# ISAE-PNX/SaDVIO

Hardware: AMD Instinct MI355X
Metric: BA iterations/sec (ms/solve in ms_per_solve), 20-KF/8k-landmark window (higher is better)
Workload: dtype f64; 1 GPU; synthetic 20 KF x 8000 landmarks x 40000 reprojection factors (pixel), GN 10 iters (LM step attempts, early exits disabled); windows_per_gpu=1, parallelism=single window, n_kf=20, n_lmk=8000, n_obs=40000, reduced_dim=114

## Files before the change

### sadvio_amd/csrc/ba_types.h

```cpp
#pragma once
#include <stdint.h>

namespace sadvio {

struct SolveOpts {
    int max_num_iterations;
    int jacobi_scaling;
    int max_num_consecutive_invalid_steps;
    int pad;
    double function_tolerance, gradient_tolerance, parameter_tolerance;
    double initial_radius, max_radius, min_radius;
    double min_lm_diagonal, max_lm_diagonal, min_relative_decrease;
    double huber_a;
    double max_time_ticks;
};

struct WinDev {
    int n_kf, n_cam, n_lmk, n_obs;
    int kf_base, cam_base, lmk_base, obs_base;
    int n_free_kf, dpf, Np, Npose;
    long long S_off;
    int red_off;
    int tile_begin, tile_end;
    int prior_begin, prior_end;
// ... 35 lines not shown
    double T_prior[12];
    double inf[6];
};

struct ImuDev {
    int kf_i, kf_j;
    double dt;
    double dR[9], dv[3], dp[3];
    double J_dR_bg[9], J_dv_ba[9], J_dv_bg[9], J_dp_ba[9], J_dp_bg[9];
    double W[81];
    double sa, sg;
    int win, pad;
};
struct SparseDev {
    int type, kf, lmk0, lmk1;
    int win, kf2;
    double T_prior[12], v_prior[3], ba_prior[3], bg_prior[3], delta[3];
    double W[225];
};
struct LineDev {
    double T[12], model[6];
    int col;
    int win;
};
struct LineObsDev {
    int line, kf, cam, win;
    double meas[6];
};
constexpr int LINE_ROW = 4 * 12 + 4 + 2;
constexpr int SPARSE_NE = 136, SPARSE_E_G = 120, SPARSE_E_COST = 135;
constexpr int SPARSE_H = 15 * 15 + 15 + 2;
constexpr int SPARSE_IX = SPARSE_H + SPARSE_NE;
constexpr int SPARSE_COL = SPARSE_IX + SPARSE_NE;
constexpr int SPARSE_J = SPARSE_COL + 16;
constexpr int IMU_J = 9 * 24 + 9;
constexpr int IMU_NE = 355;
constexpr int IMU_E_G = 300, IMU_E_BH = 324, IMU_E_BG = 342, IMU_E_COST = 354;
constexpr int IMU_H = IMU_J + 6;
constexpr int IMU_IX = IMU_H + IMU_NE;
constexpr int IMU_META = IMU_IX + IMU_NE;
constexpr int IMU_ROW = IMU_META + 5;

struct LmState {
    double radius, decrease_factor, x_cost, x_norm, initial_cost;
    int cur;
    int done, termination, iter;
    int n_success, n_unsuccess, n_invalid, pad;
};

struct FinalRec {
    LmState s;
    double fixed_cost;
};

struct IterAcc {
    double lin_cost;
    double cand_cost;
    double mcc;
    double step_norm2;
    double cand_norm2;
    double fixed_cost;
    unsigned long long gmax_bits;
    int chol_fail;
    int time_up;
};

struct TileAcc {
    double lin_cost, fixed_cost, gmax;
    double cand_cost, mcc, step_norm2, cand_norm2;
    double pad;
};

constexpr int BUILD_THREADS = 256;
constexpr int BUILD_WAVES = BUILD_THREADS / 64;
constexpr int MAX_TILE_KF = 24;
constexpr int MAX_TILE_FREE_KF = 20;
constexpr int MAX_GEMM_FREE_KF = 5;
constexpr int MAX_WIN_CAM = 8;
constexpr int STAGE_VALS = 18;
constexpr int MAX_LMK_OBS = 64;
constexpr int SOLVE_THREADS = 512;
constexpr int SOLVE_KFC_STRIDE = 32;
constexpr int SOLVE_KFC = 32;
constexpr int PRIOR_LIN = 28;
constexpr int PRE_KF = 8;
constexpr int PRE_MAX_TILES = 1024;
constexpr int MAX_LDS_NP = 174;

}
```

### sadvio_amd/csrc/device_math.h

```cpp
#pragma once
#include <hip/hip_runtime.h>

namespace sadvio {

struct V3 {
    double x, y, z;
};

__device__ __forceinline__ void m3_mul(const double* A, const double* B, double* C) {
#pragma unroll
    for (int i = 0; i < 3; i++)
#pragma unroll
        for (int j = 0; j < 3; j++) C[3 * i + j] = A[3 * i] * B[j] + A[3 * i + 1] * B[3 + j] + A[3 * i + 2] * B[6 + j];
}
__device__ __forceinline__ void m3_vec(const double* A, const double* v, double* o) {
    double x = A[0] * v[0] + A[1] * v[1] + A[2] * v[2];
    double y = A[3] * v[0] + A[4] * v[1] + A[5] * v[2];
    double z = A[6] * v[0] + A[7] * v[1] + A[8] * v[2];
    o[0] = x; o[1] = y; o[2] = z;
}
__device__ __forceinline__ void m3_tvec(const double* A, const double* v, double* o) {
    double x = A[0] * v[0] + A[3] * v[1] + A[6] * v[2];
    double y = A[1] * v[0] + A[4] * v[1] + A[7] * v[2];
    double z = A[2] * v[0] + A[5] * v[1] + A[8] * v[2];
// ... 131 lines not shown
__device__ __forceinline__ void li_vec(const double* Li, const double* t, double* u) {
    u[0] = Li[0] * t[0];
    u[1] = Li[1] * t[0] + Li[2] * t[1];
    u[2] = Li[3] * t[0] + Li[4] * t[1] + Li[5] * t[2];
}
__device__ __forceinline__ void li_tvec(const double* Li, const double* u, double* v) {
    v[0] = Li[0] * u[0] + Li[1] * u[1] + Li[3] * u[2];
    v[1] = Li[2] * u[1] + Li[4] * u[2];
    v[2] = Li[5] * u[2];
}
__device__ __forceinline__ void m3_inverse(const double* A, double* I) {
    double c00 = A[4] * A[8] - A[5] * A[7];
    double c01 = A[5] * A[6] - A[3] * A[8];
    double c02 = A[3] * A[7] - A[4] * A[6];
    double id = 1.0 / (A[0] * c00 + A[1] * c01 + A[2] * c02);
    I[0] = c00 * id; I[1] = (A[2] * A[7] - A[1] * A[8]) * id; I[2] = (A[1] * A[5] - A[2] * A[4]) * id;
    I[3] = c01 * id; I[4] = (A[0] * A[8] - A[2] * A[6]) * id; I[5] = (A[2] * A[3] - A[0] * A[5]) * id;
    I[6] = c02 * id; I[7] = (A[1] * A[6] - A[0] * A[7]) * id; I[8] = (A[0] * A[4] - A[1] * A[3]) * id;
}

__device__ __forceinline__ void relative_pose_factor(const double* Ta, const double* Tb, const double* Tab, const double* W,
                                                     const double* da, const double* db, double* r, double* J) {
    double Ea[9], Eb[9], Rau[9], Rbu[9], tau[3], tbu[3], v[3];
    so3_exp(da, Ea); so3_exp(db, Eb);
    m3_mul(Ta, Ea, Rau); m3_mul(Tb, Eb, Rbu);
    m3_vec(Ta, da + 3, v); for (int i = 0; i < 3; i++) tau[i] = v[i] + Ta[9 + i];
    m3_vec(Tb, db + 3, v); for (int i = 0; i < 3; i++) tbu[i] = v[i] + Tb[9 + i];
    double RaT_Rb[9], R[9], d[3], u[3], t[3], w[3];
    m3_tmul(Rau, Rbu, RaT_Rb);
    m3_tmul(Tab, RaT_Rb, R);
    for (int i = 0; i < 3; i++) d[i] = tbu[i] - tau[i];
    m3_tvec(Rau, d, u);
    for (int i = 0; i < 3; i++) u[i] -= Tab[9 + i];
    m3_tvec(Tab, u, t);
    so3_log(R, w);
    const double e[6] = {w[0], w[1], w[2], t[0], t[1], t[2]};
    for (int i = 0; i < 6; i++) { double s = 0.0; for (int j = 0; j < 6; j++) s += W[6 * i + j] * e[j]; r[i] = s; }
    if (!J) return;
    double Jrw[9], Jrwi[9], Jra[9], Jrb[9], A[9], B[9], C[9], S[9], D1[9], D2[9], D3[9], D4[9], E2[9], F[9];
    so3_right_jacobian(w, Jrw); m3_inverse(Jrw, Jrwi);
    so3_right_jacobian(da, Jra); so3_right_jacobian(db, Jrb);
    m3_tmul(Rbu, Rau, A); m3_mul(Jrwi, A, B); m3_mul(B, Jra, C);
    so3_skew(d, S);
    for (int i = 0; i < 3; i++) for (int j = 0; j < 3; j++) { double s = 0.0; for (int k = 0; k < 3; k++) s += Tab[3 * k + i] * Rau[3 * j + k]; D1[3 * i + j] = s; }
    m3_mul(D1, S, D2); m3_mul(D2, Rau, D3); m3_mul(D3, Jra, D4);
    m3_mul(Jrwi, Jrb, E2);
    m3_mul(D1, Rbu, F);
    double Jf[72];
    for (int i = 0; i < 72; i++) Jf[i] = 0.0;
    for (int i = 0; i < 3; i++)
        for (int j = 0; j < 3; j++) {
            Jf[i * 12 + j] = -C[3 * i + j];
            Jf[(3 + i) * 12 + j] = D4[3 * i + j];
            Jf[(3 + i) * 12 + 3 + j] = -Tab[3 * j + i];
            Jf[i * 12 + 6 + j] = E2[3 * i + j];
            Jf[(3 + i) * 12 + 9 + j] = F[3 * i + j];
        }
    for (int i = 0; i < 6; i++)
        for (int c = 0; c < 15; c++) {
            double s = 0.0;
            if (c < 12) for (int k = 0; k < 6; k++) s += W[6 * i + k] * Jf[k * 12 + c];
            J[i * 15 + c] = s;
        }
}

constexpr int POSE_TAB = 42;
__device__ __forceinline__ void pose_table_entry(const double* T0, const double* d6, double* tab) {
    double dR[9], Jr[9], R[9], t[3];
    so3_exp(d6, dR);
    so3_right_jacobian(d6, Jr);
    m3_mul(T0, dR, R);
    m3_vec(T0, d6 + 3, t);
#pragma unroll
    for (int i = 0; i < 9; i++) {
        tab[i] = R[i];
        tab[12 + i] = Jr[i];
        tab[21 + i] = T0[i];
        tab[30 + i] = dR[i];
    }
    tab[9] = t[0] + T0[9]; tab[10] = t[1] + T0[10]; tab[11] = t[2] + T0[11];
    tab[39] = d6[3]; tab[40] = d6[4]; tab[41] = d6[5];
}

template <bool WANT_J>
__device__ __forceinline__ void p2l_pseudo_obs(const double* tab, const double* q, const double* delta, const double* W, int half,
                                               double* r, double* Jp, double* Jl) {
    double Rq[3], e[3];
    m3_vec(tab, q, Rq);
    for (int a = 0; a < 3; a++) e[a] = Rq[a] + tab[9 + a] - delta[a];
    const int r0 = half ? 2 : 0;
    r[0] = W[3 * r0] * e[0] + W[3 * r0 + 1] * e[1] + W[3 * r0 + 2] * e[2];
    r[1] = half ? 0.0 : W[3] * e[0] + W[4] * e[1] + W[5] * e[2];
    if (WANT_J) {
        double Sq[9], A[9], B[9], C[9], WR0[9], WR[9];
        so3_skew(q, Sq);
        m3_mul(tab + 30, Sq, A);
        m3_mul(A, tab + 12, B);
        m3_mul(W, tab + 21, WR0);
        m3_mul(WR0, B, C);
        m3_mul(W, tab, WR);
#pragma unroll
        for (int j = 0; j < 3; j++) {
            Jp[j] = -C[3 * r0 + j]; Jp[3 + j] = WR0[3 * r0 + j]; Jl[j] = WR[3 * r0 + j];
            Jp[6 + j] = half ? 0.0 : -C[3 + j]; Jp[9 + j] = half ? 0.0 : WR0[3 + j]; Jl[3 + j] = half ? 0.0 : WR[3 + j];
        }
    }
}

template <bool WANT_J>
__device__ __forceinline__ bool pixel_factor(const double* tab, const double* K, const double* Tsf, const double* pw,
                                             double u_meas, double v_meas, double inv_sigma, double* r, double* Jp,
                                             double* Jl) {
    double pf[3], tc[3];
    m3_vec(tab, pw, pf);
    pf[0] += tab[9]; pf[1] += tab[10]; pf[2] += tab[11];
    m3_vec(Tsf, pf, tc);
    tc[0] += Tsf[9]; tc[1] += Tsf[10]; tc[2] += Tsf[11];
    double iz = 1.0 / tc[2];
    double u = (K[0] * tc[0] + K[2] * tc[2]) * iz;
    double v = (K[1] * tc[1] + K[3] * tc[2]) * iz;
    bool valid = !(tc[2] < 0.1) && !(u < 0 || v < 0 || u > 2 * K[2] || v > 2 * K[3]) && isfinite(u) && isfinite(v);
    r[0] = valid ? inv_sigma * (u - u_meas) : 0.0;
    r[1] = valid ? inv_sigma * (v - v_meas) : 0.0;
    if (WANT_J) {
        double a0 = inv_sigma * K[0] * iz, a1 = inv_sigma * K[1] * iz;
        double JhK[6] = {a0, 0.0, -a0 * tc[0] * iz, 0.0, a1, -a1 * tc[1] * iz};
        double A[6];
#pragma unroll
        for (int j = 0; j < 3; j++) {
            A[j] = JhK[0] * Tsf[j] + JhK[2] * Tsf[6 + j];
            A[3 + j] = JhK[4] * Tsf[3 + j] + JhK[5] * Tsf[6 + j];
        }
#pragma unroll
        for (int q = 0; q < 2; q++)
#pragma unroll
            for (int j = 0; j < 3; j++) Jl[3 * q + j] = A[3 * q] * tab[j] + A[3 * q + 1] * tab[3 + j] + A[3 * q + 2] * tab[6 + j];
        const double* Jr = tab + 12;
        const double* R0 = tab + 21;
#pragma unroll
        for (int q = 0; q < 2; q++) {
            double l0 = Jl[3 * q], l1 = Jl[3 * q + 1], l2 = Jl[3 * q + 2];
            double s0 = l1 * pw[2] - l2 * pw[1];
            double s1 = l2 * pw[0] - l0 * pw[2];
            double s2 = l0 * pw[1] - l1 * pw[0];
#pragma unroll
            for (int j = 0; j < 3; j++) {
                Jp[6 * q + j] = -(s0 * Jr[j] + s1 * Jr[3 + j] + s2 * Jr[6 + j]);
                Jp[6 * q + 3 + j] = A[3 * q] * R0[j] + A[3 * q + 1] * R0[3 + j] + A[3 * q + 2] * R0[6 + j];
            }
        }
    }
    return valid;
}

template <bool WANT_J>
__device__ __forceinline__ void angular_factor(const double* tab, const double* Tsf, const double* pw,
                                               const double* b, double inv_sigma, double* r, double* Jp, double* Jl) {
    const double* R0 = tab + 21;
    const double* dR = tab + 30;
    double pf[3], ts[3];
    m3_vec(tab, pw, pf);
    pf[0] += tab[9]; pf[1] += tab[10]; pf[2] += tab[11];
    m3_vec(Tsf, pf, ts);
    ts[0] += Tsf[9]; ts[1] += Tsf[10]; ts[2] += Tsf[11];
    double nrm = v3_norm(ts);
    double inrm = 1.0 / nrm;
// ... 388 lines not shown
```

### sadvio_amd/csrc/kernels.h

```cpp
#pragma once
#include "ba_types.h"
#include "device_math.h"
#include "chol16.h"

namespace sadvio {

struct DevPtrs {
    const WinDev* win;
    const Tile* tiles;
    const double* kf_T0;
    const int* kf_fidx;
    double* xp; double* xv; double* xba; double* xbg;
    long long xp_stride, xv_stride, xl_stride;
    const double* kf_vel; const double* kf_ba; const double* kf_bg;
    const double* cam_K; const double* cam_T; const double* cam_isig;
    const double* lmk_p; double* xl; double* s_lmk;
    const unsigned char* lmk_const;
    const int* lmk_ob; const int* lmk_oe;
    const int* obs_kf; const int* obs_cam; const double* obs_meas;
    const unsigned char* obs_slot;
    const int* tile_kf;
    const int* tile_row;
    const int4* pre_lane;
    const int2* pre_kf;
// ... 1119 lines not shown
                                              const double* xba, const double* xbg, const double* xl, const double* y,
                                              double* r, double* J) {
    const int fi = f.kf >= 0 ? P.kf_fidx[f.kf] : -1;
    const int lr0 = sparse_lr0(P, W, f);
    const int lr1 = (f.lmk1 >= 0 && P.lmk_red) ? P.lmk_red[f.lmk1] : -1;
    if (fi < 0 && lr0 < 0 && lr1 < 0) return false;
    const int dpf = W.dpf;
    if (f.type == 5) {
        double da[6], db[6];
        for (int q = 0; q < 6; q++) {
            da[q] = xp[6 * (long long)f.kf + q] + ((y && fi >= 0) ? y[fi * dpf + q] : 0.0);
            db[q] = xp[6 * (long long)f.kf2 + q] + ((y && lr0 >= 0) ? y[lr0 + q] : 0.0);
        }
        relative_pose_factor(P.kf_T0 + 12 * (long long)f.kf, P.kf_T0 + 12 * (long long)f.kf2, f.T_prior, f.W, da, db, r, J);
        return true;
    }
    if (f.type == 0) {
        double prm[15];
        const long long k = f.kf;
        for (int q = 0; q < 6; q++) prm[q] = xp[6 * k + q] + ((y && fi >= 0) ? y[fi * dpf + q] : 0.0);
        for (int q = 0; q < 3; q++) {
            const bool st = y && fi >= 0 && dpf == 15;
            prm[6 + q] = xv[3 * k + q] + (st ? y[fi * 15 + 6 + q] : 0.0);
            prm[9 + q] = xba[3 * k + q] + (st ? y[fi * 15 + 9 + q] : 0.0);
            prm[12 + q] = xbg[3 * k + q] + (st ? y[fi * 15 + 12 + q] : 0.0);
        }
        if (INL) imu_prior_factor_body(P.kf_T0 + 12 * k, P.kf_vel + 3 * k, P.kf_ba + 3 * k, P.kf_bg + 3 * k, f.T_prior, f.v_prior,
                                       f.ba_prior, f.bg_prior, f.W, prm, r, J);
        else imu_prior_factor(P.kf_T0 + 12 * k, P.kf_vel + 3 * k, P.kf_ba + 3 * k, P.kf_bg + 3 * k, f.T_prior, f.v_prior,
                              f.ba_prior, f.bg_prior, f.W, prm, r, J);
        return true;
    }
    double q0[3], q1[3] = {0.0, 0.0, 0.0};
    for (int a = 0; a < 3; a++) {
        q0[a] = P.lmk_p[3 * (long long)f.lmk0 + a] + xl[3 * (long long)f.lmk0 + a] + ((y && lr0 >= 0) ? y[lr0 + a] : 0.0);
        if (f.type == 3) q1[a] = P.lmk_p[3 * (long long)f.lmk1 + a] + xl[3 * (long long)f.lmk1 + a] + ((y && lr1 >= 0) ? y[lr1 + a] : 0.0);
    }
    if (f.type == 1) {
        double d6[6];
        for (int q = 0; q < 6; q++) d6[q] = xp[6 * (long long)f.kf + q] + ((y && fi >= 0) ? y[fi * dpf + q] : 0.0);
        pose_to_landmark_factor(P.kf_T0 + 12 * (long long)f.kf, q0, f.delta, f.W, d6, r, J);
        return true;
    }
    double e[3];
    for (int a = 0; a < 3; a++) e[a] = q0[a] - q1[a] - f.delta[a];
    m3_vec(f.W, e, r);
    if (J) {
        for (int i = 0; i < 3; i++)
            for (int j = 0; j < 3; j++) { J[i * 15 + j] = f.W[3 * i + j]; J[i * 15 + 3 + j] = -f.W[3 * i + j]; }
    }
    return true;
}

__device__ __noinline__ bool sparse_eval(const DevPtrs& P, const WinDev& W, const SparseDev& f, const double* xp, const double* xv,
                                        const double* xba, const double* xbg, const double* xl, const double* y,
                                        double* r, double* J) {
    return sparse_eval_t<false>(P, W, f, xp, xv, xba, xbg, xl, y, r, J);
}


__device__ __forceinline__ double prior_lin_record(const double* T0, const double* Tp, const double* inf, const double* d6, double* rec) {
    double r[6], J[36];
    pose_prior_factor(T0, Tp, inf, d6, r, J);
    double c = 0.0;
#pragma unroll
    for (int a = 0; a < 6; a++) {
        c += r[a] * r[a];
        double g = 0.0;
#pragma unroll
        for (int q = 0; q < 6; q++) g += J[6 * q + a] * r[q];
        rec[a] = g;
#pragma unroll
        for (int b = 0; b <= a; b++) {
            double hh = 0.0;
#pragma unroll
            for (int q = 0; q < 6; q++) hh += J[6 * q + a] * J[6 * q + b];
            rec[6 + a * (a + 1) / 2 + b] = hh;
        }
    }
    rec[27] = c;
    return c;
}

__device__ __noinline__ void pose_table_store(const double* T0, double d0, double d1, double d2, double d3, double d4, double d5, double* dst) {
    double T0r[12], tab[POSE_TAB];
#pragma unroll
    for (int i = 0; i < 12; i++) T0r[i] = T0[i];
    const double d6[6] = {d0, d1, d2, d3, d4, d5};
    pose_table_entry(T0r, d6, tab);
#pragma unroll
    for (int i = 0; i < POSE_TAB; i++) dst[i] = tab[i];
}
__device__ __noinline__ double prior_lin_record_call(const double* T0, double d0, double d1, double d2, double d3, double d4, double d5, const PriorDev* pr,
                                                     double* rec) {
    double T0r[12];
#pragma unroll
    for (int i = 0; i < 12; i++) T0r[i] = T0[i];
    const double d6[6] = {d0, d1, d2, d3, d4, d5};
    const PriorDev q = *pr;
    return prior_lin_record(T0r, q.T_prior, q.inf, d6, rec);
}

template <int MODE, bool EXTRAS>
__global__ __launch_bounds__(SOLVE_THREADS) void k_solve(DevPtrs P, int slot) {
    extern __shared__ __attribute__((aligned(16))) char smem[];
    constexpr bool BIG = MODE != 0;
    const int w = blockIdx.x;
    const WinDev W = P.win[w];
    if (BIG != (W.ld != 0)) return;
    const int tid = threadIdx.x;
    const int wv = __builtin_amdgcn_readfirstlane(tid >> 6), ln = tid & 63, nwv = blockDim.x >> 6;
    LmState* stp = P.states + (long long)w * P.state_stride + slot;
    IterAcc* acc = P.acc + (long long)w * P.state_stride + slot;
    __shared__ int s_done;
    __shared__ double s_red[SOLVE_THREADS / 64 * 4];
    SADVIO_TS(3, 0);
#ifdef SADVIO_KERNEL_TS
    if ((P.debug & 4096) && blockIdx.x == 0 && tid == 0 && slot == 3) P.dbg_ts[20] = clock64();
#endif
    LmState st = *stp;
    if (MODE == 1 && tid == 0) P.big_info[w] = 0;
    if (st.done) return;
    const int Np = W.Np;
    const long long ld = W.ld;
    double* Sg = P.S + W.S_off;
    double* gredg = P.gred + W.red_off;
    double* gfullg = P.gfull + W.red_off;
    double* hdg = P.hdiag + W.red_off;
    const int nbt = c16_blocks(Np + 1);
    const int img_n = c16_size(Np);
    double* A = BIG ? Sg : (double*)smem;
    double* y = BIG ? gredg : A + img_n;
    double* gf = BIG ? gfullg : y + Np;
    double* hd = BIG ? hdg : gf + Np;
    double* xs = BIG ? gredg : hd + Np;
    double* pub = xs + Np + (Np & 1);
    double* yv = pub + C16_WORK;
    double* kfc = yv + 16 * nbt;
    auto aidx = [&](int i, int j) -> long long { return BIG ? (long long)i * ld + j : (long long)c16_index(i, j); };
    const int cur = st.cur;
    const double* xp = P.xp + (long long)cur * P.xp_stride;
    const int n_imu = W.imu_end - W.imu_begin;
    double early_cost = 0.0, early_fixed = 0.0, early_gm = 0.0;
    double cost_part = 0.0, fixed_part = 0.0;
    const int n_pri = W.prior_end - W.prior_begin;
    const double* plin = P.prior_lin + (long long)cur * P.prior_lin_stride + (long long)W.prior_begin * PRIOR_LIN;
    double pl_v = 0.0;
    int pl_fi = -1;
    if (MODE != 2 && tid < n_pri * 28) {
        const int p = tid / 28, e = tid - 28 * p;
        pl_v = plin[p * PRIOR_LIN + e];
        pl_fi = P.kf_fidx[P.priors[W.prior_begin + p].kf];
    }
    double* sp = P.s_pose + W.red_off;
    double c_sp = 1.0;
    const bool det = P.world > 1;
    if (MODE != 2) {
    double im_ix[8], im_v[8];
    const int n_imu_items = (EXTRAS && !det && !P.imu_direct) ? n_imu * IMU_NE : 0;
    if (EXTRAS) {
#pragma unroll
        for (int u = 0; u < 8; u++) {
            const int it = tid + u * (int)blockDim.x;
            im_ix[u] = -1.0; im_v[u] = 0.0;
            if (it < n_imu_items) {
                const int k = it / IMU_NE, e = it - IMU_NE * k;
                const double* row = P.imu_scratch + (long long)cur * P.imu_scratch_stride + (long long)(W.imu_begin + k) * IMU_ROW;
                im_ix[u] = row[IMU_IX + e]; im_v[u] = row[IMU_H + e];
            }
        }
    }
    if (!BIG) {
        typedef __attribute__((address_space(3))) void lds_void_t;
        typedef __attribute__((address_space(1))) const void glb_void_t;
// ... 232 lines not shown
        if (tid < Np) {
            gm = fmax(gm, fabs(gf[tid]));
            const double hdi = hd[tid];
            double s = c_sp;
            if (slot == 0) { s = P.o.jacobi_scaling ? 1.0 / (1.0 + sqrt(hdi)) : 1.0; sp[tid] = s; }
            const double s2 = s * s;
            A[c16_index(tid, tid)] += fmin(fmax(s2 * hdi, P.o.min_lm_diagonal), P.o.max_lm_diagonal) / st.radius / s2;
            A[c16_index(Np, tid)] = y[tid];
        }
    } else {
        for (int i = tid; i < Np; i += blockDim.x) gm = fmax(gm, fabs(gf[i]));
    }
    gm = wave_max(gm); cost_part = wave_sum(cost_part); fixed_part = wave_sum(fixed_part);
    if (ln == 0) { s_red[wv * 3] = gm; s_red[wv * 3 + 1] = cost_part; s_red[wv * 3 + 2] = fixed_part; }
    if (tid == 0) s_done = 0;
    __syncthreads();
    if (!BIG) c16_symmetrize(A, nbt);
    if (tid == blockDim.x - 1) {
        double g = 0, cs = 0, fs = 0;
        for (int k = 0; k < nwv; k++) { g = fmax(g, s_red[k * 3]); cs += s_red[k * 3 + 1]; fs += s_red[k * 3 + 2]; }
        acc->gmax_bits = (unsigned long long)__double_as_longlong(g);
        acc->lin_cost = cs;
        acc->fixed_cost = fs;
        acc->cand_cost = 0.0; acc->mcc = 0.0; acc->step_norm2 = 0.0; acc->cand_norm2 = 0.0;
        const bool time_up = P.o.max_time_ticks > 0.0 && P.t_start && (double)(wall_clock64() - *P.t_start) >= P.o.max_time_ticks;
        acc->time_up = time_up ? 1 : 0;
        const bool no_iterations = st.iter == 0 && P.o.max_num_iterations <= 0;
        if (time_up || g <= P.o.gradient_tolerance || no_iterations) {
            LmState e = st;
            e.done = 1; e.termination = (time_up || g > P.o.gradient_tolerance) ? 0 : 3;
            e.x_cost = 0.5 * cs;
            if (e.iter == 0) e.initial_cost = e.x_cost;
            *stp = e;
            s_done = 1;
        }
    }
    __syncthreads();
    if (s_done) return;
    SADVIO_TS(3, 2);
    if (BIG) {
        for (int i = tid; i < Np; i += blockDim.x) {
            double s;
            if (slot == 0) { s = P.o.jacobi_scaling ? 1.0 / (1.0 + sqrt(hd[i])) : 1.0; sp[i] = s; }
            else s = sp[i];
            double s2 = s * s;
            A[aidx(i, i)] += fmin(fmax(s2 * hd[i], P.o.min_lm_diagonal), P.o.max_lm_diagonal) / st.radius / s2;
        }
        __syncthreads();
    }
    SADVIO_TS(3, 3);
    if (MODE == 1) return;
    }
    long long* ts = SADVIO_TS_PTR((P.debug & 4096) && blockIdx.x == 0 && slot == 3);
    if (MODE == 0) {
        bool ok = true;
        if (Np > 0) ok = c16_solve<1>(A, Np, xs, pub, yv, ts ? ts + 64 : nullptr);
        if (!ok) {
            if (tid == 0) acc->chol_fail = 1;
            return;
        }
    } else {
        y = P.delta + W.red_off;
        if (P.big_info[w] != 0) {
            for (int i = tid; i < Np; i += blockDim.x) { gredg[i] = 0.0; gfullg[i] = 0.0; hdg[i] = 0.0; }
            if (tid == 0) acc->chol_fail = 1;
            return;
        }
    }
    SADVIO_TS(3, 4);
    double* dl = P.delta + W.red_off;
    double sn = 0.0, cn = 0.0;
    bool bad = false;
    for (int i = tid; i < Np; i += blockDim.x) {
        double d = -xs[i];
        dl[i] = d;
        y[i] = d;
        sn += d * d;
        if (!isfinite(d)) bad = true;
        if (BIG) { gredg[i] = 0.0; gfullg[i] = 0.0; hdg[i] = 0.0; }
    }
    __syncthreads();
    SADVIO_TS(3, 5);
    double* xpc = P.xp + (long long)(1 - cur) * P.xp_stride;
    for (int k = tid; k < W.n_kf; k += blockDim.x) {
        int g = W.kf_base + k;
        const bool pre = MODE == 0 && k < SOLVE_KFC;
        const double* kc = kfc + (pre ? k : 0) * SOLVE_KFC_STRIDE;
        int fi = pre ? (int)kc[0] : P.kf_fidx[g];
        double d6[6];
        const double* T0r = pre ? kc + 7 : P.kf_T0 + 12 * (long long)g;
        double vbb[9];
        if (W.dpf == 15) {
            const double* xs3[3] = {P.xv + (long long)cur * P.xv_stride, P.xba + (long long)cur * P.xv_stride, P.xbg + (long long)cur * P.xv_stride};
#pragma unroll
            for (int q = 0; q < 3; q++)
#pragma unroll
                for (int i = 0; i < 3; i++) vbb[3 * q + i] = pre ? kc[19 + 3 * q + i] : xs3[q][3 * (long long)g + i];
        }
#pragma unroll
        for (int i = 0; i < 6; i++) {
            double v = (pre ? kc[1 + i] : xp[6 * (long long)g + i]) + (fi < 0 ? 0.0 : y[fi * W.dpf + i]);
            xpc[6 * (long long)g + i] = v;
            d6[i] = v;
            if (fi >= 0) cn += v * v;
        }
        pose_table_store(T0r, d6[0], d6[1], d6[2], d6[3], d6[4], d6[5], P.ptab + (long long)(1 - cur) * P.ptab_stride + (long long)g * POSE_TAB);
        if (W.dpf == 15) {
            double* xs3[3] = {P.xv + (long long)(1 - cur) * P.xv_stride, P.xba + (long long)(1 - cur) * P.xv_stride, P.xbg + (long long)(1 - cur) * P.xv_stride};
#pragma unroll
            for (int q = 0; q < 3; q++)
#pragma unroll
                for (int i = 0; i < 3; i++) {
                    const double v = vbb[3 * q + i] + (fi < 0 ? 0.0 : y[fi * 15 + 6 + 3 * q + i]);
                    xs3[q][3 * (long long)g + i] = v;
                    if (fi >= 0) cn += v * v;
                }
        }
    }
    if (EXTRAS && W.line_end > W.line_begin) {
        const double* xlc = P.xline + (long long)cur * P.xline_stride;
        double* xln = P.xline + (long long)(1 - cur) * P.xline_stride;
        for (int it = tid; it < (W.line_end - W.line_begin) * 6; it += blockDim.x) {
            const int l = W.line_begin + it / 6, q = it % 6;
            const int lc = P.lines[l].col;
            const double v = xlc[6 * (long long)l + q] + (lc < 0 ? 0.0 : y[lc + q]);
            xln[6 * (long long)l + q] = v;
            if (lc >= 0) cn += v * v;
        }
    }
    SADVIO_TS(3, 6);
    double mcc = 0.0, cc = 0.0;
    {
        const double* plx = P.prior_lin + (long long)cur * P.prior_lin_stride + (long long)W.prior_begin * PRIOR_LIN;
        double* plc = P.prior_lin + (long long)(1 - cur) * P.prior_lin_stride + (long long)W.prior_begin * PRIOR_LIN;
        for (int p = (int)blockDim.x - 1 - tid; p < W.prior_end - W.prior_begin; p += blockDim.x) {
            const PriorDev* prp = P.priors + W.prior_begin + p;
            const int pkf = prp->kf;
            const int fi = P.kf_fidx[pkf];
            if (fi < 0) continue;
            double d[6], d6[6];
#pragma unroll
            for (int i = 0; i < 6; i++) { d[i] = y[fi * W.dpf + i]; d6[i] = xp[6 * (long long)pkf + i] + d[i]; }
            double lin = 0.0, quad = 0.0;
#pragma unroll
            for (int a = 0; a < 6; a++) {
                lin += d[a] * plx[p * PRIOR_LIN + a];
#pragma unroll
                for (int b = 0; b <= a; b++) quad += (a == b ? 0.5 : 1.0) * d[a] * d[b] * plx[p * PRIOR_LIN + 6 + a * (a + 1) / 2 + b];
            }
            mcc += -(lin + quad);
            cc += prior_lin_record_call(P.kf_T0 + 12 * (long long)pkf, d6[0], d6[1], d6[2], d6[3], d6[4], d6[5], prp, plc + p * PRIOR_LIN);
        }
    }
    if (EXTRAS && n_imu > 0) {
        const double* xv = P.xv + (long long)cur * P.xv_stride;
        const double* xba = P.xba + (long long)cur * P.xv_stride;
        const double* xbg = P.xbg + (long long)cur * P.xv_stride;
        const int t0 = blockDim.x > 128 ? 64 : 0;
        for (int it = tid - t0; it >= 0 && it < n_imu * 15; it += blockDim.x - t0) {
            const int k = it / 15, q = it - 15 * k;
            const double* sc = P.imu_scratch + (long long)cur * P.imu_scratch_stride + (long long)(W.imu_begin + k) * IMU_ROW;
            const int fi = (int)sc[IMU_META], fj = (int)sc[IMU_META + 1];
            if (fi < 0 && fj < 0) continue;
            double m = 0.0, r;
            if (q < 9) {
                double jr[24];
#pragma unroll
                for (int a = 0; a < 24; a++) jr[a] = sc[q * 24 + a];
                r = sc[9 * 24 + q];
#pragma unroll
                for (int a = 0; a < 24; a++) { const int ca = imu_col(a, fi, fj); if (ca >= 0) m += jr[a] * y[ca]; }
            } else {
                const int e = q - 9, ax = e % 3, gy = e / 3;
                const double sgm = sc[IMU_META + 2 + gy];
                r = sc[IMU_J + e];
                if (fi >= 0) m -= sgm * y[fi * 15 + 9 + 3 * gy + ax];
                if (fj >= 0) m += sgm * y[fj * 15 + 9 + 3 * gy + ax];
            }
            mcc += -m * (r + 0.5 * m);
        }
    }
    if (EXTRAS && W.spl_end > W.spl_begin) {
        const int t0 = blockDim.x > 320 ? 256 : 0;
        for (int it = tid - t0; it >= 0 && it < (W.spl_end - W.spl_begin) * 15; it += blockDim.x - t0) {
            const int kl = it / 15, q = it - 15 * kl;
            const double* sc = P.sp_scratch + (long long)cur * P.sp_scratch_stride + (long long)P.sp_list[W.spl_begin + kl] * SPARSE_J;
            if (q >= (int)sc[SPARSE_COL + 15]) continue;
            double jr[15], cd[15];
#pragma unroll
            for (int a = 0; a < 15; a++) { jr[a] = sc[q * 15 + a]; cd[a] = sc[SPARSE_COL + a]; }
            const double r = sc[225 + q];
            double m = 0.0;
#pragma unroll
            for (int a = 0; a < 15; a++) { const int ca = (int)cd[a]; if (ca >= 0) m += jr[a] * y[ca]; }
            mcc += -m * (r + 0.5 * m);
        }
    }
    if (EXTRAS && W.lobs_end > W.lobs_begin) {
        const int rows = W.factor_type == 0 ? 4 : 2;
        for (int it = tid; it < (W.lobs_end - W.lobs_begin) * 4; it += blockDim.x) {
            const int k = it >> 2, q = it & 3;
            if (q >= rows) continue;
            const LineObsDev& ob = P.lobs[W.lobs_begin + k];
            const int fi = P.kf_fidx[ob.kf], lc = P.lines[ob.line].col;
            if (fi < 0 && lc < 0) continue;
            const double* sc = P.line_scratch + (long long)(W.lobs_begin + k) * LINE_ROW;
            double m = 0.0;
            for (int a = 0; a < 6; a++) {
                if (fi >= 0) m += sc[q * 12 + a] * y[fi * W.dpf + a];
                if (lc >= 0) m += sc[q * 12 + 6 + a] * y[lc + a];
            }
            mcc += -m * (sc[48 + q] + 0.5 * m);
        }
    }
    SADVIO_TS(3, 7);
    sn = wave_sum(sn); cn = wave_sum(cn); mcc = wave_sum(mcc); cc = wave_sum(cc);
    if (bad) acc->chol_fail = 1;
    __syncthreads();
    if (ln == 0) { s_red[wv * 4] = sn; s_red[wv * 4 + 1] = cn; s_red[wv * 4 + 2] = mcc; s_red[wv * 4 + 3] = cc; }
    __syncthreads();
    if (tid == 0) {
        double a0 = 0, a1 = 0, a2 = 0, a3 = 0;
        for (int k = 0; k < nwv; k++) { a0 += s_red[k * 4]; a1 += s_red[k * 4 + 1]; a2 += s_red[k * 4 + 2]; a3 += s_red[k * 4 + 3]; }
        acc->step_norm2 = a0; acc->cand_norm2 = a1; acc->mcc = a2; acc->cand_cost = a3;
    }
    SADVIO_TS(3, 8);
    if (ts && tid == 0) { ts[15] = wall_clock64(); ts[21] = clock64(); }
}


__device__ __forceinline__ void zero_s_slice(const DevPtrs& P, const Tile& T, int tile_index) {
    if (T.ld != 0) return;
    const int n2 = c16_size(T.Np) >> 1;
    const int per = (n2 + T.win_ntiles - 1) / T.win_ntiles;
    const int i0 = (tile_index - T.win_tile0) * per, i1 = min(i0 + per, n2);
    double2* S2 = (double2*)(P.S + T.S_off);
    const double2 z2 = make_double2(0.0, 0.0);
    for (int i = i0 + (int)threadIdx.x; i < i1; i += blockDim.x) S2[i] = z2;
}

template <int FACTOR, bool RARE, bool IMU>
__global__ __launch_bounds__(BUILD_THREADS) void k_backsub(DevPtrs P, int slot, int max_tile_kf) {
    extern __shared__ __attribute__((aligned(16))) char smem[];
    if (IMU && (int)blockIdx.x >= P.n_tiles) {
        if (threadIdx.x < 64) pose_factor_eval<true>(P, slot, (int)blockIdx.x - P.n_tiles, threadIdx.x);
        return;
    }
    const Tile T = P.tiles[blockIdx.x];
    const int tid = threadIdx.x, wv = tid >> 6, ln = tid & 63;
    int4 pl = make_int4(0, -1, 0, 0);
    int2 pk = make_int2(-1, -1), pk6 = make_int2(-1, -1);
    if (P.pre_lane) {
        pl = P.pre_lane[(long long)blockIdx.x * (BUILD_THREADS / 8) + (tid >> 3)];
        pk = P.pre_kf[(long long)blockIdx.x * PRE_KF + tid / POSE_TAB];
        if (tid < PRE_KF * 6) pk6 = P.pre_kf[(long long)blockIdx.x * PRE_KF + tid / 6];
    }
    LmState st;
    int chol_fail;
    if (P.n_win == 1) { st = P.states[slot]; chol_fail = P.acc[slot].chol_fail; }
    else { st = P.states[(long long)T.w * P.state_stride + slot]; chol_fail = P.acc[(long long)T.w * P.state_stride + slot].chol_fail; }
    zero_s_slice(P, T, blockIdx.x);
    double* poseTab = (double*)smem;
    double* camTab = poseTab + (size_t)max_tile_kf * POSE_TAB;
    int* rowTab = (int*)(camTab + MAX_WIN_CAM * 17);
    double* candTab = (double*)(smem + tile_tables_bytes(max_tile_kf));
    double* dpTab = candTab + (size_t)max_tile_kf * 12;
    const int G = T.G, lpw = 64 / G;
    const int grp = ln / G, q = ln - grp * G;
    const int nl = T.lmk1 - T.lmk0;
    bool first_valid;
    int gl_first, pre_ob, pre_oe, pre_o;
    if (P.pre_lane) {
        first_valid = (pl.z >> 16) & 1; gl_first = pl.x; pre_ob = pl.y; pre_oe = pl.y + (pl.z & 0xff);
        pre_o = (pl.w + (tid & 7) < (pl.z & 0xff)) ? pl.y + pl.w + (tid & 7) : -1;
    } else {
        first_valid = wv * lpw + grp < nl;
        gl_first = T.lmk0 + (first_valid ? wv * lpw + grp : 0);
        pre_ob = P.lmk_ob[gl_first]; pre_oe = P.lmk_oe[gl_first];
        pre_o = (first_valid && q < pre_oe - pre_ob) ? pre_ob + q : -1;
    }
    const int pre_lcode = P.lmk_const ? P.lmk_const[gl_first] : 0;
    double pre_p[3], pre_xa[3], pre_xb[3];
#pragma unroll
    for (int i = 0; i < 3; i++) {
        pre_p[i] = P.lmk_p[3 * (long long)gl_first + i];
        pre_xa[i] = P.xl[3 * (long long)gl_first + i];
        pre_xb[i] = P.xl[P.xl_stride + 3 * (long long)gl_first + i];
    }
    ObsPre pre_obs;
    pre_obs.slot = 0; pre_obs.craw = 0; pre_obs.m[0] = pre_obs.m[1] = pre_obs.m[2] = 0.0;
    if (pre_o >= 0) pre_obs = obs_prefetch<FACTOR>(P, pre_o);
    double pre_t0 = 0.0, pre_t1 = 0.0;
    const bool pre_tab = P.pre_lane != nullptr;
    if (pre_tab && pk.x >= 0) {
        const long long src = (long long)pk.x * POSE_TAB + (tid - (tid / POSE_TAB) * POSE_TAB);
        pre_t0 = P.ptab[src]; pre_t1 = P.ptab[P.ptab_stride + src];
    }
    if (st.done || chol_fail) {
        if (tid == 0) {
            TileAcc* ta = P.tacc + (long long)(slot & 1) * P.n_tiles + blockIdx.x;
            ta->cand_cost = 0.0; ta->mcc = 0.0; ta->step_norm2 = 0.0; ta->cand_norm2 = 0.0;
        }
// ... 1068 lines not shown
```

Baseline: 18070 BA iterations/s.

## Split pose-table update into per-KF scalar stage and block-parallel element expansion

Instead of each thread serially computing and storing the full 42-entry pose table for one keyframe, each thread now computes a compact 14-scalar record (axis, sin/cos terms, Jacobian coefficients) into shared scratch. The block then expands the tables in parallel, one element per thread, and the final chunk is deferred until after the reduction so it overlaps other work. The aim is to spread the serial per-KF exp/Jacobian work across all 512 threads and coalesce the table writes. The cost is extra syncthreads, recomputed skew products per element, and shared-memory staging.

```diff
diff --git a/sadvio_amd/csrc/ba_types.h b/sadvio_amd/csrc/ba_types.h
--- a/sadvio_amd/csrc/ba_types.h
+++ b/sadvio_amd/csrc/ba_types.h
@@ -141,6 +141,7 @@
 constexpr int SOLVE_THREADS = 512;
 constexpr int SOLVE_KFC_STRIDE = 32;
 constexpr int SOLVE_KFC = 32;
+constexpr int SOLVE_REC = 32;
 constexpr int PRIOR_LIN = 28;
 constexpr int PRE_KF = 8;
 constexpr int PRE_MAX_TILES = 1024;
diff --git a/sadvio_amd/csrc/device_math.h b/sadvio_amd/csrc/device_math.h
--- a/sadvio_amd/csrc/device_math.h
+++ b/sadvio_amd/csrc/device_math.h
@@ -237,6 +237,58 @@
     tab[39] = d6[3]; tab[40] = d6[4]; tab[41] = d6[5];
 }
 
+constexpr int POSE_REC = 14;
+__device__ __forceinline__ void pose_table_scalars(const double* d6, double* rec) {
+    const double n = v3_norm(d6);
+    const bool exp_first_order = n < 1e-9, jr_identity = n < 1e-5;
+    double ax[3] = {d6[0], d6[1], d6[2]}, c = 0.0, s = 0.0, a = 0.0, b = 0.0;
+    if (!exp_first_order) {
+        ax[0] = d6[0] / n; ax[1] = d6[1] / n; ax[2] = d6[2] / n;
+        double sn, cs;
+        sincos_f64(n, &sn, &cs);
+        c = 1. - cs; s = sn;
+        if (!jr_identity) { a = (1 - cs) / (n * n); b = (n - sn) / (n * n * n); }
+    }
+#pragma unroll
+    for (int i = 0; i < 6; i++) rec[i] = d6[i];
+    rec[6] = ax[0]; rec[7] = ax[1]; rec[8] = ax[2];
+    rec[9] = c; rec[10] = s; rec[11] = a; rec[12] = b;
+    rec[13] = (double)((exp_first_order ? 1 : 0) | (jr_identity ? 2 : 0));
+}
+__device__ __forceinline__ double so3_skew_at(const double* u, int i, int j) {
+    if (i == j) return 0.0;
+    const double v = u[3 - i - j];
+    return (j - i == 1 || j - i == -2) ? -v : v;
+}
+__device__ __forceinline__ double so3_skew2_at(const double* u, int i, int j) {
+    return so3_skew_at(u, i, 0) * so3_skew_at(u, 0, j) + so3_skew_at(u, i, 1) * so3_skew_at(u, 1, j) + so3_skew_at(u, i, 2) * so3_skew_at(u, 2, j);
+}
+__device__ __forceinline__ double pose_rec_dR(const double* rec, int i, int j) {
+    double r = i == j ? 1.0 : 0.0;
+    if ((int)rec[13] & 1) r += so3_skew_at(rec, i, j);
+    else r += rec[9] * so3_skew2_at(rec + 6, i, j) + rec[10] * so3_skew_at(rec + 6, i, j);
+    return r;
+}
+__device__ __forceinline__ double pose_rec_Jr(const double* rec, int i, int j) {
+    const double r = i == j ? 1.0 : 0.0;
+    if ((int)rec[13] & 2) return r;
+    return r - rec[11] * so3_skew_at(rec, i, j) + rec[12] * so3_skew2_at(rec, i, j);
+}
+__device__ __forceinline__ double pose_table_item(const double* T0, const double* rec, int e) {
+    if (e < 9) {
+        const int i = e / 3, j = e - 3 * i;
+        return T0[3 * i] * pose_rec_dR(rec, 0, j) + T0[3 * i + 1] * pose_rec_dR(rec, 1, j) + T0[3 * i + 2] * pose_rec_dR(rec, 2, j);
+    }
+    if (e < 12) {
+        const int i = e - 9;
+        return (T0[3 * i] * rec[3] + T0[3 * i + 1] * rec[4] + T0[3 * i + 2] * rec[5]) + T0[9 + i];
+    }
+    if (e < 21) return pose_rec_Jr(rec, (e - 12) / 3, (e - 12) % 3);
+    if (e < 30) return T0[e - 21];
+    if (e < 39) return pose_rec_dR(rec, (e - 30) / 3, (e - 30) % 3);
+    return rec[e - 36];
+}
+
 template <bool WANT_J>
 __device__ __forceinline__ void p2l_pseudo_obs(const double* tab, const double* q, const double* delta, const double* W, int half,
                                                double* r, double* Jp, double* Jl) {
diff --git a/sadvio_amd/csrc/kernels.h b/sadvio_amd/csrc/kernels.h
--- a/sadvio_amd/csrc/kernels.h
+++ b/sadvio_amd/csrc/kernels.h
@@ -1225,14 +1225,9 @@
     return c;
 }
 
-__device__ __noinline__ void pose_table_store(const double* T0, double d0, double d1, double d2, double d3, double d4, double d5, double* dst) {
-    double T0r[12], tab[POSE_TAB];
-#pragma unroll
-    for (int i = 0; i < 12; i++) T0r[i] = T0[i];
+__device__ __noinline__ void pose_scalars_store(double d0, double d1, double d2, double d3, double d4, double d5, double* rec) {
     const double d6[6] = {d0, d1, d2, d3, d4, d5};
-    pose_table_entry(T0r, d6, tab);
-#pragma unroll
-    for (int i = 0; i < POSE_TAB; i++) dst[i] = tab[i];
+    pose_table_scalars(d6, rec);
 }
 __device__ __noinline__ double prior_lin_record_call(const double* T0, double d0, double d1, double d2, double d3, double d4, double d5, const PriorDev* pr,
                                                      double* rec) {
@@ -1631,40 +1626,73 @@
     __syncthreads();
     SADVIO_TS(3, 5);
     double* xpc = P.xp + (long long)(1 - cur) * P.xp_stride;
-    for (int k = tid; k < W.n_kf; k += blockDim.x) {
-        int g = W.kf_base + k;
-        const bool pre = MODE == 0 && k < SOLVE_KFC;
-        const double* kc = kfc + (pre ? k : 0) * SOLVE_KFC_STRIDE;
-        int fi = pre ? (int)kc[0] : P.kf_fidx[g];
-        double d6[6];
-        const double* T0r = pre ? kc + 7 : P.kf_T0 + 12 * (long long)g;
-        double vbb[9];
-        if (W.dpf == 15) {
-            const double* xs3[3] = {P.xv + (long long)cur * P.xv_stride, P.xba + (long long)cur * P.xv_stride, P.xbg + (long long)cur * P.xv_stride};
-#pragma unroll
-            for (int q = 0; q < 3; q++)
-#pragma unroll
-                for (int i = 0; i < 3; i++) vbb[3 * q + i] = pre ? kc[19 + 3 * q + i] : xs3[q][3 * (long long)g + i];
-        }
-#pragma unroll
-        for (int i = 0; i < 6; i++) {
-            double v = (pre ? kc[1 + i] : xp[6 * (long long)g + i]) + (fi < 0 ? 0.0 : y[fi * W.dpf + i]);
-            xpc[6 * (long long)g + i] = v;
-            d6[i] = v;
-            if (fi >= 0) cn += v * v;
-        }
-        pose_table_store(T0r, d6[0], d6[1], d6[2], d6[3], d6[4], d6[5], P.ptab + (long long)(1 - cur) * P.ptab_stride + (long long)g * POSE_TAB);
+    __shared__ double s_rec[MODE == 2 ? SOLVE_KFC * SOLVE_REC : 1];
+    double* recs = MODE == 0 ? A : s_rec;
+    const int rec_cap = MODE == 0 ? img_n / SOLVE_REC : SOLVE_KFC;
+    auto stage_e = [&](int k0, int k1) {
+        const int nk = k1 - k0;
+        const long long g0 = W.kf_base + k0;
+        double* tabc = P.ptab + (long long)(1 - cur) * P.ptab_stride + g0 * POSE_TAB;
+        for (int it = tid; it < nk * POSE_TAB; it += blockDim.x) {
+            const int kk = it / POSE_TAB, e = it - POSE_TAB * kk;
+            const double* rec = recs + kk * SOLVE_REC;
+            tabc[it] = (MODE == 0 && k0 + kk < SOLVE_KFC) ? pose_table_item(kfc + (k0 + kk) * SOLVE_KFC_STRIDE + 7, rec, e)
+                                                          : pose_table_item(P.kf_T0 + 12 * (g0 + kk), rec, e);
+        }
+        const int rt = (int)blockDim.x - 1 - tid;
+        for (int it = rt; it < nk * 6; it += blockDim.x) xpc[6 * g0 + it] = recs[(it / 6) * SOLVE_REC + it % 6];
         if (W.dpf == 15) {
             double* xs3[3] = {P.xv + (long long)(1 - cur) * P.xv_stride, P.xba + (long long)(1 - cur) * P.xv_stride, P.xbg + (long long)(1 - cur) * P.xv_stride};
-#pragma unroll
-            for (int q = 0; q < 3; q++)
-#pragma unroll
-                for (int i = 0; i < 3; i++) {
-                    const double v = vbb[3 * q + i] + (fi < 0 ? 0.0 : y[fi * 15 + 6 + 3 * q + i]);
-                    xs3[q][3 * (long long)g + i] = v;
-                    if (fi >= 0) cn += v * v;
-                }
-        }
+            for (int it = rt; it < nk * 9; it += blockDim.x) {
+                const int q = it / (3 * nk), r = it - 3 * nk * q;
+                xs3[q][3 * g0 + r] = recs[(r / 3) * SOLVE_REC + 16 + 3 * q + r % 3];
+            }
+        }
+    };
+    int ke0 = 0;
+    for (;;) {
+        const int ke1 = min(ke0 + rec_cap, W.n_kf);
+        for (int k = tid; k < ke1; k += blockDim.x) {
+            if (k < ke0) continue;
+            int g = W.kf_base + k;
+            const bool pre = MODE == 0 && k < SOLVE_KFC;
+            const double* kc = kfc + (pre ? k : 0) * SOLVE_KFC_STRIDE;
+            int fi = pre ? (int)kc[0] : P.kf_fidx[g];
+            double d6[6];
+            double vbb[9];
+            if (W.dpf == 15) {
+                const double* xs3[3] = {P.xv + (long long)cur * P.xv_stride, P.xba + (long long)cur * P.xv_stride, P.xbg + (long long)cur * P.xv_stride};
+#pragma unroll
+                for (int q = 0; q < 3; q++)
+#pragma unroll
+                    for (int i = 0; i < 3; i++) vbb[3 * q + i] = pre ? kc[19 + 3 * q + i] : xs3[q][3 * (long long)g + i];
+            }
+#pragma unroll
+            for (int i = 0; i < 6; i++) {
+                double v = (pre ? kc[1 + i] : xp[6 * (long long)g + i]) + (fi < 0 ? 0.0 : y[fi * W.dpf + i]);
+                d6[i] = v;
+                if (fi >= 0) cn += v * v;
+            }
+            SADVIO_TS(3, 9);
+            double* rec = recs + (k - ke0) * SOLVE_REC;
+            pose_scalars_store(d6[0], d6[1], d6[2], d6[3], d6[4], d6[5], rec);
+            SADVIO_TS(3, 10);
+            if (W.dpf == 15) {
+#pragma unroll
+                for (int q = 0; q < 3; q++)
+#pragma unroll
+                    for (int i = 0; i < 3; i++) {
+                        const double v = vbb[3 * q + i] + (fi < 0 ? 0.0 : y[fi * 15 + 6 + 3 * q + i]);
+                        rec[16 + 3 * q + i] = v;
+                        if (fi >= 0) cn += v * v;
+                    }
+            }
+        }
+        if (ke1 >= W.n_kf) break;
+        __syncthreads();
+        stage_e(ke0, ke1);
+        __syncthreads();
+        ke0 = ke1;
     }
     if (EXTRAS && W.line_end > W.line_begin) {
         const double* xlc = P.xline + (long long)cur * P.xline_stride;
@@ -1767,6 +1795,9 @@
     if (bad) acc->chol_fail = 1;
     __syncthreads();
     if (ln == 0) { s_red[wv * 4] = sn; s_red[wv * 4 + 1] = cn; s_red[wv * 4 + 2] = mcc; s_red[wv * 4 + 3] = cc; }
+    SADVIO_TS(3, 11);
+    stage_e(ke0, W.n_kf);
+    SADVIO_TS(3, 12);
     __syncthreads();
     if (tid == 0) {
         double a0 = 0, a1 = 0, a2 = 0, a3 = 0;
```

Result: slower. 16730 BA iterations/s (-7.4%).
